# Zokrates/ZoKrates

Measured on NVIDIA H100. Metric: groth16_constraints_per_sec, higher is better.
Workload: dtype u256-montgomery

## Files before the change

zokrates_b200/csrc/ec.cuh:

```cuda
#pragma once
#include "fp2.cuh"

namespace zkb {

template <class F>
struct Affine {
  F x, y;
  ZKB_HD bool is_inf() const { return x.is_zero() && y.is_zero(); }
  ZKB_HD static Affine inf() { return Affine{F::zero(), F::zero()}; }
  ZKB_HD static Affine neg(const Affine& p) { return Affine{p.x, F::neg(p.y)}; }
};

template <class F>
struct XYZZ {
  F x, y, zz, zzz;

  ZKB_HD static XYZZ identity() { return XYZZ{F::zero(), F::zero(), F::zero(), F::zero()}; }
  ZKB_HD bool is_identity() const { return zz.is_zero(); }
  ZKB_HD static XYZZ from_affine(const Affine<F>& p) {
    if (p.is_inf()) return identity();
    return XYZZ{p.x, p.y, F::one(), F::one()};
  }
  ZKB_HD static XYZZ neg(const XYZZ& p) { return XYZZ{p.x, F::neg(p.y), p.zz, p.zzz}; }

  ZKB_HD static XYZZ mdbl(const Affine<F>& p) {
    F U = F::dbl(p.y);
    F V = F::sqr(U);
    F W = F::mul(U, V);
    F S = F::mul(p.x, V);
    F X2 = F::sqr(p.x);
    F M = F::add(F::dbl(X2), X2);
    F X3 = F::sub(F::sqr(M), F::dbl(S));
    F Y3 = F::sub(F::mul(M, F::sub(S, X3)), F::mul(W, p.y));
    return XYZZ{X3, Y3, V, W};
  }

  ZKB_HD static XYZZ dbl(const XYZZ& p) {
    F U = F::dbl(p.y);
    F V = F::sqr(U);
    F W = F::mul(U, V);
    F S = F::mul(p.x, V);
    F X2 = F::sqr(p.x);
    F M = F::add(F::dbl(X2), X2);
    F X3 = F::sub(F::sqr(M), F::dbl(S));
    F Y3 = F::sub(F::mul(M, F::sub(S, X3)), F::mul(W, p.y));
    return XYZZ{X3, Y3, F::mul(V, p.zz), F::mul(W, p.zzz)};
  }

  ZKB_HD static XYZZ madd(const XYZZ& a, const Affine<F>& q) {
    if (q.is_inf()) return a;
    if (a.is_identity()) return XYZZ{q.x, q.y, F::one(), F::one()};
    F U2 = F::mul(q.x, a.zz);
    F S2 = F::mul(q.y, a.zzz);
    F Pd = F::sub(U2, a.x);
    F Rd = F::sub(S2, a.y);
    if (Pd.is_zero()) {
      if (Rd.is_zero()) return mdbl_ni(q);
      return identity();
    }
    F PP = F::sqr(Pd);
    F PPP = F::mul(Pd, PP);
    F Q = F::mul(a.x, PP);
    F X3 = F::sub(F::sub(F::sqr(Rd), PPP), F::dbl(Q));
    F Y3 = F::sub(F::mul(Rd, F::sub(Q, X3)), F::mul(a.y, PPP));
    return XYZZ{X3, Y3, F::mul(a.zz, PP), F::mul(a.zzz, PPP)};
  }

  ZKB_HD static XYZZ add(const XYZZ& a, const XYZZ& b) {
    if (b.is_identity()) return a;
    if (a.is_identity()) return b;
    F U1 = F::mul(a.x, b.zz);
    F U2 = F::mul(b.x, a.zz);
    F S1 = F::mul(a.y, b.zzz);
    F S2 = F::mul(b.y, a.zzz);
    F Pd = F::sub(U2, U1);
    F Rd = F::sub(S2, S1);
    if (Pd.is_zero()) {
      if (Rd.is_zero()) return dbl_ni(a);
      return identity();
    }
    F PP = F::sqr(Pd);
    F PPP = F::mul(Pd, PP);
    F Q = F::mul(U1, PP);
    F X3 = F::sub(F::sub(F::sqr(Rd), PPP), F::dbl(Q));
    F Y3 = F::sub(F::mul(Rd, F::sub(Q, X3)), F::mul(S1, PPP));
    return XYZZ{X3, Y3, F::mul(F::mul(a.zz, b.zz), PP), F::mul(F::mul(a.zzz, b.zzz), PPP)};
  }

  ZKB_NI static XYZZ mdbl_ni(const Affine<F>& p) { return mdbl(p); }
  ZKB_NI static XYZZ dbl_ni(const XYZZ& p) { return dbl(p); }
  ZKB_NI static XYZZ add_ni(const XYZZ& a, const XYZZ& b) { return add(a, b); }
  ZKB_NI static XYZZ madd_ni(const XYZZ& a, const Affine<F>& q) { return madd(a, q); }

  ZKB_NI static Affine<F> to_affine(const XYZZ& p) {
    if (p.is_identity()) return Affine<F>::inf();
    F t = F::inv(F::mul(p.zz, p.zzz));
    F zzi = F::mul(t, p.zzz);
    F zzzi = F::mul(t, p.zz);
    return Affine<F>{F::mul(p.x, zzi), F::mul(p.y, zzzi)};
  }

  ZKB_NI static XYZZ mul_affine(const Affine<F>& base, const uint32_t* k, int nlimbs) {
    XYZZ r = identity();
    for (int i = nlimbs - 1; i >= 0; i--)
      for (int b = 31; b >= 0; b--) {
        r = dbl_ni(r);
        if ((k[i] >> b) & 1) r = madd_ni(r, base);
      }
    return r;
  }
  ZKB_NI static XYZZ mul_xyzz(const XYZZ& base, const uint32_t* k, int nlimbs) {
    XYZZ r = identity();
    for (int i = nlimbs - 1; i >= 0; i--)
      for (int b = 31; b >= 0; b--) {
        r = dbl_ni(r);
        if ((k[i] >> b) & 1) r = add_ni(r, base);
      }
    return r;
  }
};

}
```

zokrates_b200/csrc/fp.cuh:

```cuda
#pragma once
#include "hd.cuh"
#include "field_params.cuh"

namespace zkb {

template <class P>
struct alignas(16) Fp {
  static constexpr int N = P::N;
  typedef P Params;
  uint32_t v[N];

  ZKB_HD static Fp zero() {
    Fp r;
#pragma unroll
    for (int i = 0; i < N; i++) r.v[i] = 0;
    return r;
  }
  ZKB_HD static Fp one() {
    Fp r;
#pragma unroll
    for (int i = 0; i < N; i++) r.v[i] = P::r1(i);
    return r;
  }
  ZKB_HD static Fp r2() {
    Fp r;
#pragma unroll
    for (int i = 0; i < N; i++) r.v[i] = P::r2(i);
    return r;
  }
  ZKB_HD static Fp modulus() {
    Fp r;
#pragma unroll
    for (int i = 0; i < N; i++) r.v[i] = P::mod(i);
    return r;
  }
  ZKB_HD bool is_zero() const {
    uint32_t acc = 0;
#pragma unroll
    for (int i = 0; i < N; i++) acc |= v[i];
    return acc == 0;
  }
  ZKB_HD bool operator==(const Fp& o) const {
    uint32_t acc = 0;
#pragma unroll
    for (int i = 0; i < N; i++) acc |= v[i] ^ o.v[i];
    return acc == 0;
  }
  ZKB_HD bool operator!=(const Fp& o) const { return !(*this == o); }

  ZKB_HD static Fp reduce_once(const Fp& a) {
    Fp t;
    t.v[0] = ptx::sub_cc(a.v[0], P::mod(0));
#pragma unroll
    for (int i = 1; i < N; i++) t.v[i] = ptx::subc_cc(a.v[i], P::mod(i));
    uint32_t borrow = ptx::subc(0, 0);
    Fp r;
#pragma unroll
    for (int i = 0; i < N; i++) r.v[i] = borrow ? a.v[i] : t.v[i];
    return r;
  }

  ZKB_HD static Fp add(const Fp& a, const Fp& b) {
    Fp t;
    t.v[0] = ptx::add_cc(a.v[0], b.v[0]);
#pragma unroll
    for (int i = 1; i < N - 1; i++) t.v[i] = ptx::addc_cc(a.v[i], b.v[i]);
    t.v[N - 1] = ptx::addc(a.v[N - 1], b.v[N - 1]);
    return reduce_once(t);
  }

  ZKB_HD static Fp sub(const Fp& a, const Fp& b) {
    Fp t;
    t.v[0] = ptx::sub_cc(a.v[0], b.v[0]);
#pragma unroll
    for (int i = 1; i < N; i++) t.v[i] = ptx::subc_cc(a.v[i], b.v[i]);
    uint32_t borrow = ptx::subc(0, 0);
    Fp r;
    r.v[0] = ptx::add_cc(t.v[0], P::mod(0) & borrow);
#pragma unroll
    for (int i = 1; i < N - 1; i++) r.v[i] = ptx::addc_cc(t.v[i], P::mod(i) & borrow);
    r.v[N - 1] = ptx::addc(t.v[N - 1], P::mod(N - 1) & borrow);
    return r;
  }

  ZKB_HD static Fp neg(const Fp& a) {
    if (a.is_zero()) return a;
    Fp r;
    r.v[0] = ptx::sub_cc(P::mod(0), a.v[0]);
#pragma unroll
    for (int i = 1; i < N - 1; i++) r.v[i] = ptx::subc_cc(P::mod(i), a.v[i]);
    r.v[N - 1] = ptx::subc(P::mod(N - 1), a.v[N - 1]);
    return r;
  }

  ZKB_HD static Fp dbl(const Fp& a) { return add(a, a); }

  ZKB_HD static Fp mul(const Fp& a, const Fp& b) {
    static_assert(N % 2 == 0, "even limb count");
    uint32_t E[N], O[N];
    {
      const uint32_t y = b.v[0];
#pragma unroll
      for (int j = 0; j < N; j += 2) {
        uint64_t w = (uint64_t)a.v[j] * y;
        E[j] = (uint32_t)w;
        E[j + 1] = (uint32_t)(w >> 32);
        uint64_t u = (uint64_t)a.v[j + 1] * y;
        O[j] = (uint32_t)u;
        O[j + 1] = (uint32_t)(u >> 32);
      }
    }
#pragma unroll
    for (int i = 0; i < N; i++) {
      if (i > 0) {
        const uint32_t y = b.v[i];
        uint32_t nE[N], nO[N];
        nE[0] = ptx::add_cc(O[0], E[1]);
#pragma unroll
        for (int j = 1; j < N - 1; j += 2) ptx::madc_wide_cc(nO[j - 1], nO[j], a.v[j], y, E[j + 1], E[j + 2]);
        ptx::madc_wide(nO[N - 2], nO[N - 1], a.v[N - 1], y, 0, 0);
        ptx::mad_wide_cc(nE[0], nE[1], a.v[0], y, nE[0], O[1]);
#pragma unroll
        for (int j = 2; j < N; j += 2) ptx::madc_wide_cc(nE[j], nE[j + 1], a.v[j], y, O[j], O[j + 1]);
        nO[N - 1] = ptx::addc(nO[N - 1], 0);
#pragma unroll
        for (int j = 0; j < N; j++) {
          E[j] = nE[j];
          O[j] = nO[j];
        }
      }
      const uint32_t m = E[0] * P::INV;
      ptx::mad_wide_cc(O[0], O[1], P::mod(1), m, O[0], O[1]);
#pragma unroll
      for (int j = 3; j < N; j += 2) ptx::madc_wide_cc(O[j - 1], O[j], P::mod(j), m, O[j - 1], O[j]);
      ptx::mad_wide_cc(E[0], E[1], P::mod(0), m, E[0], E[1]);
#pragma unroll
      for (int j = 2; j < N; j += 2) ptx::madc_wide_cc(E[j], E[j + 1], P::mod(j), m, E[j], E[j + 1]);
      O[N - 1] = ptx::addc(O[N - 1], 0);
    }
    Fp t;
    t.v[0] = ptx::add_cc(O[0], E[1]);
#pragma unroll
    for (int k = 1; k < N - 1; k++) t.v[k] = ptx::addc_cc(O[k], E[k + 1]);
    t.v[N - 1] = ptx::addc(O[N - 1], 0);
    return reduce_once(t);
  }

  ZKB_HD static Fp sqr(const Fp& a) { return mul(a, a); }
  ZKB_NI static Fp mul_ni(const Fp& a, const Fp& b) { return mul(a, b); }

  ZKB_HD static Fp to_mont(const Fp& a) { return mul(a, r2()); }
  ZKB_HD static Fp from_mont(const Fp& a) {
    Fp o = zero();
    o.v[0] = 1;
    return mul(a, o);
  }

  ZKB_NI static Fp pow_limbs(const Fp& a, const uint32_t* e, int nlimbs) {
    Fp r = one();
    bool started = false;
    for (int i = nlimbs - 1; i >= 0; i--) {
      for (int b = 31; b >= 0; b--) {
        if (started) r = mul_ni(r, r);
        if ((e[i] >> b) & 1) {
          r = started ? mul_ni(r, a) : a;
          started = true;
        }
      }
    }
    return r;
  }

  ZKB_NI static Fp inv(const Fp& a) {
    uint32_t e[N];
#pragma unroll
    for (int i = 0; i < N; i++) e[i] = P::pm2(i);
    return pow_limbs(a, e, N);
  }

  ZKB_NI static Fp pow_u64(const Fp& a, uint64_t k) {
    uint32_t e[2] = {(uint32_t)k, (uint32_t)(k >> 32)};
    return pow_limbs(a, e, 2);
  }
};

}
```

zokrates_b200/csrc/fp2.cuh:

```cuda
#pragma once
#include "fp.cuh"

namespace zkb {

template <class Bt>
struct Fp2T {
  typedef Bt B;
  typedef Fp2T Fp2;
  B c0, c1;

  ZKB_HD static Fp2 zero() { return Fp2{B::zero(), B::zero()}; }
  ZKB_HD static Fp2 one() { return Fp2{B::one(), B::zero()}; }
  ZKB_HD bool is_zero() const { return c0.is_zero() && c1.is_zero(); }
  ZKB_HD bool operator==(const Fp2& o) const { return c0 == o.c0 && c1 == o.c1; }
  ZKB_HD bool operator!=(const Fp2& o) const { return !(*this == o); }
  ZKB_HD static Fp2 add(const Fp2& a, const Fp2& b) { return Fp2{B::add(a.c0, b.c0), B::add(a.c1, b.c1)}; }
  ZKB_HD static Fp2 sub(const Fp2& a, const Fp2& b) { return Fp2{B::sub(a.c0, b.c0), B::sub(a.c1, b.c1)}; }
  ZKB_HD static Fp2 neg(const Fp2& a) { return Fp2{B::neg(a.c0), B::neg(a.c1)}; }
  ZKB_HD static Fp2 dbl(const Fp2& a) { return Fp2{B::dbl(a.c0), B::dbl(a.c1)}; }
  ZKB_NI static Fp2 mul_v(Fp2 a, Fp2 b) {
    B v0 = B::mul(a.c0, b.c0);
    B v1 = B::mul(a.c1, b.c1);
    B s = B::mul(B::add(a.c0, a.c1), B::add(b.c0, b.c1));
    return Fp2{B::sub(v0, v1), B::sub(B::sub(s, v0), v1)};
  }
  ZKB_NI static Fp2 sqr_v(Fp2 a) {
    B t = B::mul(a.c0, a.c1);
    B r0 = B::mul(B::add(a.c0, a.c1), B::sub(a.c0, a.c1));
    return Fp2{r0, B::dbl(t)};
  }
  ZKB_HD static Fp2 mul(const Fp2& a, const Fp2& b) { return mul_v(a, b); }
  ZKB_HD static Fp2 sqr(const Fp2& a) { return sqr_v(a); }
  ZKB_HD static Fp2 mul_ni(const Fp2& a, const Fp2& b) { return mul_v(a, b); }
  ZKB_NI static Fp2 inv(const Fp2& a) {
    B d = B::inv(B::add(B::sqr(a.c0), B::sqr(a.c1)));
    return Fp2{B::mul(a.c0, d), B::neg(B::mul(a.c1, d))};
  }
  ZKB_HD static Fp2 to_mont(const Fp2& a) { return Fp2{B::to_mont(a.c0), B::to_mont(a.c1)}; }
  ZKB_HD static Fp2 from_mont(const Fp2& a) { return Fp2{B::from_mont(a.c0), B::from_mont(a.c1)}; }
};

template <class P>
using Fp2 = Fp2T<Fp<P>>;

}
```

zokrates_b200/csrc/fp64.cuh:

```cuda
#pragma once
#include "fp.cuh"

namespace zkb {

template <class P>
struct alignas(16) Fp64 {
  static constexpr int N = P::N / 2;
  typedef P Params;
  typedef unsigned __int128 u128;
  uint64_t v[N];

  ZKB_HD static uint64_t modl(int i) { return ((uint64_t)P::mod(2 * i + 1) << 32) | P::mod(2 * i); }
  ZKB_HD static uint64_t inv64() {
    uint64_t p0 = modl(0);
    uint64_t x = (uint64_t)(uint32_t)(0u - P::INV);
    x = x * (2 - p0 * x);
    return (uint64_t)0 - x;
  }
  ZKB_HD static Fp64 zero() { Fp64 r; for (int i = 0; i < N; i++) r.v[i] = 0; return r; }
  ZKB_HD static Fp64 one() { Fp64 r; for (int i = 0; i < N; i++) r.v[i] = ((uint64_t)P::r1(2 * i + 1) << 32) | P::r1(2 * i); return r; }
  ZKB_HD static Fp64 r2() { Fp64 r; for (int i = 0; i < N; i++) r.v[i] = ((uint64_t)P::r2(2 * i + 1) << 32) | P::r2(2 * i); return r; }
  ZKB_HD bool is_zero() const { uint64_t a = 0; for (int i = 0; i < N; i++) a |= v[i]; return a == 0; }
  ZKB_HD bool operator==(const Fp64& o) const { uint64_t a = 0; for (int i = 0; i < N; i++) a |= v[i] ^ o.v[i]; return a == 0; }
  ZKB_HD bool operator!=(const Fp64& o) const { return !(*this == o); }
  ZKB_HD static bool geq_p(const Fp64& a) {
    for (int i = N - 1; i >= 0; i--) { uint64_t m = modl(i); if (a.v[i] > m) return true; if (a.v[i] < m) return false; }
    return true;
  }
  ZKB_HD static Fp64 sub_p(const Fp64& a) {
    Fp64 r; uint64_t borrow = 0;
    for (int i = 0; i < N; i++) { u128 d = (u128)a.v[i] - modl(i) - borrow; r.v[i] = (uint64_t)d; borrow = (uint64_t)(d >> 64) & 1; }
    return r;
  }
  ZKB_HD static Fp64 add(const Fp64& a, const Fp64& b) {
    Fp64 t; uint64_t c = 0;
    for (int i = 0; i < N; i++) { u128 s = (u128)a.v[i] + b.v[i] + c; t.v[i] = (uint64_t)s; c = (uint64_t)(s >> 64); }
    return (c || geq_p(t)) ? sub_p(t) : t;
  }
  ZKB_HD static Fp64 sub(const Fp64& a, const Fp64& b) {
    Fp64 t; uint64_t borrow = 0;
    for (int i = 0; i < N; i++) { u128 d = (u128)a.v[i] - b.v[i] - borrow; t.v[i] = (uint64_t)d; borrow = (uint64_t)(d >> 64) & 1; }
    if (borrow) { uint64_t c = 0; for (int i = 0; i < N; i++) { u128 s = (u128)t.v[i] + modl(i) + c; t.v[i] = (uint64_t)s; c = (uint64_t)(s >> 64); } }
    return t;
  }
  ZKB_HD static Fp64 neg(const Fp64& a) { return a.is_zero() ? a : sub(zero(), a); }
  ZKB_HD static Fp64 dbl(const Fp64& a) { return add(a, a); }
  ZKB_HD static Fp64 mul(const Fp64& a, const Fp64& b) {
    uint64_t t[N + 2];
    for (int i = 0; i < N + 2; i++) t[i] = 0;
    const uint64_t inv = inv64();
    for (int i = 0; i < N; i++) {
      uint64_t c = 0;
      for (int j = 0; j < N; j++) { u128 s = (u128)a.v[j] * b.v[i] + t[j] + c; t[j] = (uint64_t)s; c = (uint64_t)(s >> 64); }
      u128 s2 = (u128)t[N] + c; t[N] = (uint64_t)s2; t[N + 1] = (uint64_t)(s2 >> 64);
      uint64_t m = t[0] * inv;
      u128 s = (u128)m * modl(0) + t[0]; c = (uint64_t)(s >> 64);
      for (int j = 1; j < N; j++) { s = (u128)m * modl(j) + t[j] + c; t[j - 1] = (uint64_t)s; c = (uint64_t)(s >> 64); }
      s2 = (u128)t[N] + c; t[N - 1] = (uint64_t)s2; t[N] = t[N + 1] + (uint64_t)(s2 >> 64);
    }
    Fp64 o; for (int i = 0; i < N; i++) o.v[i] = t[i];
    return (t[N] || geq_p(o)) ? sub_p(o) : o;
  }
  ZKB_HD static Fp64 sqr(const Fp64& a) { return mul(a, a); }
  ZKB_HD static Fp64 mul_ni(const Fp64& a, const Fp64& b) { return mul(a, b); }
  ZKB_HD static Fp64 to_mont(const Fp64& a) { return mul(a, r2()); }
  ZKB_HD static Fp64 from_mont(const Fp64& a) { Fp64 o = zero(); o.v[0] = 1; return mul(a, o); }
  ZKB_HD static Fp64 inv(const Fp64& a) {
    uint64_t e[N];
    for (int i = 0; i < N; i++) e[i] = modl(i);
    uint64_t borrow = 2;
    for (int i = 0; i < N && borrow; i++) { uint64_t o = e[i]; e[i] = o - borrow; borrow = o < borrow ? 1 : 0; }
    Fp64 r = one();
    bool started = false;
    for (int i = N - 1; i >= 0; i--)
      for (int b = 63; b >= 0; b--) {
        if (started) r = mul(r, r);
        if ((e[i] >> b) & 1) { r = started ? mul(r, a) : a; started = true; }
      }
    return r;
  }
};

}
```

Before: 49.40 million.

## Add lazy Montgomery reduction with wide products, dedicated squaring, and fused mul-sub

Splits Montgomery multiplication into a double-width product and a separate REDC, and adds a dedicated squaring that computes the cross terms once and doubles them. EC point addition computes Y3 as a single reduction of a*b - c*d, and Fp2 multiplication (Karatsuba) defers reduction using unreduced sums and a precomputed multiple of p^2. Together these save REDC passes and modular add/sub corrections in the MSM inner loops. This depends on the modulus having two spare top bits (BN254 does), and the new wide code paths add register pressure.

```diff
diff --git a/zokrates_b200/csrc/ec.cuh b/zokrates_b200/csrc/ec.cuh
--- a/zokrates_b200/csrc/ec.cuh
+++ b/zokrates_b200/csrc/ec.cuh
@@ -62,7 +62,7 @@
     F PPP = F::mul(Pd, PP);
     F Q = F::mul(a.x, PP);
     F X3 = F::sub(F::sub(F::sqr(Rd), PPP), F::dbl(Q));
-    F Y3 = F::sub(F::mul(Rd, F::sub(Q, X3)), F::mul(a.y, PPP));
+    F Y3 = F::mul_sub(Rd, F::sub(Q, X3), a.y, PPP);
     return XYZZ{X3, Y3, F::mul(a.zz, PP), F::mul(a.zzz, PPP)};
   }
 
@@ -83,7 +83,7 @@
     F PPP = F::mul(Pd, PP);
     F Q = F::mul(U1, PP);
     F X3 = F::sub(F::sub(F::sqr(Rd), PPP), F::dbl(Q));
-    F Y3 = F::sub(F::mul(Rd, F::sub(Q, X3)), F::mul(S1, PPP));
+    F Y3 = F::mul_sub(Rd, F::sub(Q, X3), S1, PPP);
     return XYZZ{X3, Y3, F::mul(F::mul(a.zz, b.zz), PP), F::mul(F::mul(a.zzz, b.zzz), PPP)};
   }
 
diff --git a/zokrates_b200/csrc/fp.cuh b/zokrates_b200/csrc/fp.cuh
--- a/zokrates_b200/csrc/fp.cuh
+++ b/zokrates_b200/csrc/fp.cuh
@@ -146,7 +146,184 @@
     return reduce_once(t);
   }
 
-  ZKB_HD static Fp sqr(const Fp& a) { return mul(a, a); }
+  static constexpr bool LAZY_HEADROOM = (P::mod(N - 1) >> 30) == 0;
+  struct Wide {
+    uint32_t v[2 * N];
+  };
+
+  template <int M>
+  struct PSq {
+    uint32_t v[2 * N];
+    ZKB_HD constexpr PSq() : v() {
+      for (int i = 0; i < N; i++) {
+        uint64_t c = 0;
+        for (int j = 0; j < N; j++) {
+          uint64_t t = (uint64_t)P::mod(i) * P::mod(j) + v[i + j] + c;
+          v[i + j] = (uint32_t)t;
+          c = t >> 32;
+        }
+        v[i + N] = (uint32_t)c;
+      }
+      uint64_t c = 0;
+      for (int k = 0; k < 2 * N; k++) {
+        uint64_t t = (uint64_t)v[k] * M + c;
+        v[k] = (uint32_t)t;
+        c = t >> 32;
+      }
+    }
+  };
+
+  template <int SIZE>
+  ZKB_HD static void mad_row(uint32_t (&acc)[SIZE], int s, const uint32_t* x, int j0, int cnt, uint32_t y) {
+#pragma unroll
+    for (int t = 0; t < cnt; t++) {
+      const int k = s + 2 * t;
+      if (t == 0)
+        ptx::mad_wide_cc(acc[k], acc[k + 1], x[j0], y, acc[k], acc[k + 1]);
+      else
+        ptx::madc_wide_cc(acc[k], acc[k + 1], x[j0 + 2 * t], y, acc[k], acc[k + 1]);
+    }
+    if (cnt > 0 && s + 2 * cnt < SIZE) acc[s + 2 * cnt] = ptx::addc(acc[s + 2 * cnt], 0);
+  }
+
+  ZKB_HD static Wide merge_eo(const uint32_t (&E)[2 * N], const uint32_t (&O)[2 * N]) {
+    Wide r;
+    r.v[0] = E[0];
+    r.v[1] = ptx::add_cc(E[1], O[0]);
+#pragma unroll
+    for (int k = 2; k < 2 * N - 1; k++) r.v[k] = ptx::addc_cc(E[k], O[k - 1]);
+    r.v[2 * N - 1] = ptx::addc(E[2 * N - 1], O[2 * N - 2]);
+    return r;
+  }
+
+  ZKB_HD static Wide mul_wide(const Fp& a, const Fp& b) {
+    static_assert(N % 2 == 0, "even limb count");
+    uint32_t E[2 * N], O[2 * N];
+#pragma unroll
+    for (int k = 0; k < 2 * N; k++) E[k] = O[k] = 0;
+#pragma unroll
+    for (int i = 0; i < N; i++) {
+      if (i % 2 == 0) {
+        mad_row(E, i, a.v, 0, N / 2, b.v[i]);
+        mad_row(O, i, a.v, 1, N / 2, b.v[i]);
+      } else {
+        mad_row(O, i - 1, a.v, 0, N / 2, b.v[i]);
+        mad_row(E, i + 1, a.v, 1, N / 2, b.v[i]);
+      }
+    }
+    return merge_eo(E, O);
+  }
+
+  ZKB_HD static Wide sqr_wide(const Fp& a) {
+    uint32_t E[2 * N], O[2 * N];
+#pragma unroll
+    for (int k = 0; k < 2 * N; k++) E[k] = O[k] = 0;
+#pragma unroll
+    for (int i = 0; i < N - 1; i++) {
+      mad_row(O, 2 * i, a.v, i + 1, (N - i) / 2, a.v[i]);
+      mad_row(E, 2 * i + 2, a.v, i + 2, (N - 1 - i) / 2, a.v[i]);
+    }
+    Wide t = merge_eo(E, O);
+    Wide r;
+    r.v[0] = 0;
+#pragma unroll
+    for (int k = 2 * N - 1; k >= 1; k--) r.v[k] = (t.v[k] << 1) | (t.v[k - 1] >> 31);
+    ptx::mad_wide_cc(r.v[0], r.v[1], a.v[0], a.v[0], r.v[0], r.v[1]);
+#pragma unroll
+    for (int i = 1; i < N; i++) ptx::madc_wide_cc(r.v[2 * i], r.v[2 * i + 1], a.v[i], a.v[i], r.v[2 * i], r.v[2 * i + 1]);
+    return r;
+  }
+
+  ZKB_HD static Fp redc(const Wide& T) {
+    uint32_t E[N], O[N];
+#pragma unroll
+    for (int j = 0; j < N; j++) {
+      E[j] = T.v[j];
+      O[j] = 0;
+    }
+    {
+      const uint32_t m = E[0] * P::INV;
+      ptx::mad_wide_cc(O[0], O[1], P::mod(1), m, O[0], O[1]);
+#pragma unroll
+      for (int j = 3; j < N; j += 2) ptx::madc_wide_cc(O[j - 1], O[j], P::mod(j), m, O[j - 1], O[j]);
+      ptx::mad_wide_cc(E[0], E[1], P::mod(0), m, E[0], E[1]);
+#pragma unroll
+      for (int j = 2; j < N; j += 2) ptx::madc_wide_cc(E[j], E[j + 1], P::mod(j), m, E[j], E[j + 1]);
+      O[N - 1] = ptx::addc(O[N - 1], 0);
+    }
+#pragma unroll
+    for (int i = 1; i < N; i++) {
+      uint32_t nE[N], nO[N];
+      nE[0] = ptx::add_cc(O[0], E[1]);
+      const uint32_t m = nE[0] * P::INV;
+#pragma unroll
+      for (int j = 1; j < N - 1; j += 2) ptx::madc_wide_cc(nO[j - 1], nO[j], P::mod(j), m, E[j + 1], E[j + 2]);
+      ptx::madc_wide(nO[N - 2], nO[N - 1], P::mod(N - 1), m, 0, 0);
+      ptx::mad_wide_cc(nE[0], nE[1], P::mod(0), m, nE[0], O[1]);
+#pragma unroll
+      for (int j = 2; j < N; j += 2) ptx::madc_wide_cc(nE[j], nE[j + 1], P::mod(j), m, O[j], O[j + 1]);
+      nO[N - 1] = ptx::addc(nO[N - 1], 0);
+#pragma unroll
+      for (int j = 0; j < N; j++) {
+        E[j] = nE[j];
+        O[j] = nO[j];
+      }
+    }
+    Fp t;
+    t.v[0] = ptx::add_cc(O[0], E[1]);
+#pragma unroll
+    for (int k = 1; k < N - 1; k++) t.v[k] = ptx::addc_cc(O[k], E[k + 1]);
+    t.v[N - 1] = ptx::addc(O[N - 1], 0);
+    t.v[0] = ptx::add_cc(t.v[0], T.v[N]);
+#pragma unroll
+    for (int k = 1; k < N - 1; k++) t.v[k] = ptx::addc_cc(t.v[k], T.v[N + k]);
+    t.v[N - 1] = ptx::addc(t.v[N - 1], T.v[2 * N - 1]);
+    return reduce_once(t);
+  }
+
+  ZKB_HD static Wide add_wide(const Wide& a, const Wide& b) {
+    Wide r;
+    r.v[0] = ptx::add_cc(a.v[0], b.v[0]);
+#pragma unroll
+    for (int k = 1; k < 2 * N - 1; k++) r.v[k] = ptx::addc_cc(a.v[k], b.v[k]);
+    r.v[2 * N - 1] = ptx::addc(a.v[2 * N - 1], b.v[2 * N - 1]);
+    return r;
+  }
+  ZKB_HD static Wide sub_wide(const Wide& a, const Wide& b) {
+    Wide r;
+    r.v[0] = ptx::sub_cc(a.v[0], b.v[0]);
+#pragma unroll
+    for (int k = 1; k < 2 * N - 1; k++) r.v[k] = ptx::subc_cc(a.v[k], b.v[k]);
+    r.v[2 * N - 1] = ptx::subc(a.v[2 * N - 1], b.v[2 * N - 1]);
+    return r;
+  }
+  template <int M>
+  ZKB_HD static Wide add_psq(const Wide& a) {
+    static_assert(LAZY_HEADROOM && M <= 2, "M p^2 plus the operand must stay < p*R");
+    constexpr PSq<M> K{};
+    Wide r;
+    r.v[0] = ptx::add_cc(a.v[0], K.v[0]);
+#pragma unroll
+    for (int i = 1; i < 2 * N - 1; i++) r.v[i] = ptx::addc_cc(a.v[i], K.v[i]);
+    r.v[2 * N - 1] = ptx::addc(a.v[2 * N - 1], K.v[2 * N - 1]);
+    return r;
+  }
+  ZKB_HD static Fp add_nr(const Fp& a, const Fp& b) {
+    static_assert(LAZY_HEADROOM, "a product of two unreduced sums (< 4p^2) must stay < p*R");
+    Fp t;
+    t.v[0] = ptx::add_cc(a.v[0], b.v[0]);
+#pragma unroll
+    for (int i = 1; i < N - 1; i++) t.v[i] = ptx::addc_cc(a.v[i], b.v[i]);
+    t.v[N - 1] = ptx::addc(a.v[N - 1], b.v[N - 1]);
+    return t;
+  }
+
+  ZKB_HD static Fp mul_sub(const Fp& a, const Fp& b, const Fp& c, const Fp& d) {
+    static_assert(LAZY_HEADROOM, "a sum of two products (< 2p^2) must stay < p*R");
+    return redc(add_wide(mul_wide(a, b), mul_wide(c, neg(d))));
+  }
+
+  ZKB_HD static Fp sqr(const Fp& a) { return redc(sqr_wide(a)); }
   ZKB_NI static Fp mul_ni(const Fp& a, const Fp& b) { return mul(a, b); }
 
   ZKB_HD static Fp to_mont(const Fp& a) { return mul(a, r2()); }
diff --git a/zokrates_b200/csrc/fp2.cuh b/zokrates_b200/csrc/fp2.cuh
--- a/zokrates_b200/csrc/fp2.cuh
+++ b/zokrates_b200/csrc/fp2.cuh
@@ -19,16 +19,42 @@
   ZKB_HD static Fp2 neg(const Fp2& a) { return Fp2{B::neg(a.c0), B::neg(a.c1)}; }
   ZKB_HD static Fp2 dbl(const Fp2& a) { return Fp2{B::dbl(a.c0), B::dbl(a.c1)}; }
   ZKB_NI static Fp2 mul_v(Fp2 a, Fp2 b) {
-    B v0 = B::mul(a.c0, b.c0);
-    B v1 = B::mul(a.c1, b.c1);
-    B s = B::mul(B::add(a.c0, a.c1), B::add(b.c0, b.c1));
-    return Fp2{B::sub(v0, v1), B::sub(B::sub(s, v0), v1)};
+    if constexpr (!B::LAZY_HEADROOM) {
+      B v0 = B::mul(a.c0, b.c0), v1 = B::mul(a.c1, b.c1);
+      B s = B::mul(B::add(a.c0, a.c1), B::add(b.c0, b.c1));
+      return Fp2{B::sub(v0, v1), B::sub(B::sub(s, v0), v1)};
+    } else {
+      typedef typename B::Wide Wd;
+      Wd v0 = B::mul_wide(a.c0, b.c0);
+      Wd v1 = B::mul_wide(a.c1, b.c1);
+      Wd s = B::mul_wide(B::add_nr(a.c0, a.c1), B::add_nr(b.c0, b.c1));
+      B c1 = B::redc(B::sub_wide(B::sub_wide(s, v0), v1));
+      B c0 = B::redc(B::sub_wide(B::template add_psq<1>(v0), v1));
+      return Fp2{c0, c1};
+    }
   }
   ZKB_NI static Fp2 sqr_v(Fp2 a) {
-    B t = B::mul(a.c0, a.c1);
-    B r0 = B::mul(B::add(a.c0, a.c1), B::sub(a.c0, a.c1));
-    return Fp2{r0, B::dbl(t)};
+    B r0 = B::mul(B::add_nr(a.c0, a.c1), B::sub(a.c0, a.c1));
+    B r1 = B::mul(B::add_nr(a.c0, a.c0), a.c1);
+    return Fp2{r0, r1};
   }
+  ZKB_NI static Fp2 mul_sub_v(Fp2 a, Fp2 b, Fp2 c, Fp2 d) {
+    if constexpr (!B::LAZY_HEADROOM) {
+      return sub(mul_v(a, b), mul_v(c, d));
+    } else {
+      typedef typename B::Wide Wd;
+      Fp2 e = neg(d);
+      Wd v0 = B::mul_wide(a.c0, b.c0);
+      Wd w0 = B::mul_wide(c.c0, e.c0);
+      Wd v1 = B::add_wide(B::mul_wide(a.c1, b.c1), B::mul_wide(c.c1, e.c1));
+      Wd s = B::add_wide(B::mul_wide(B::add_nr(a.c0, a.c1), B::add_nr(b.c0, b.c1)),
+                         B::mul_wide(B::add_nr(c.c0, c.c1), B::add_nr(e.c0, e.c1)));
+      B c1 = B::redc(B::sub_wide(B::sub_wide(B::sub_wide(s, v0), w0), v1));
+      B c0 = B::redc(B::sub_wide(B::template add_psq<2>(B::add_wide(v0, w0)), v1));
+      return Fp2{c0, c1};
+    }
+  }
+  ZKB_HD static Fp2 mul_sub(const Fp2& a, const Fp2& b, const Fp2& c, const Fp2& d) { return mul_sub_v(a, b, c, d); }
   ZKB_HD static Fp2 mul(const Fp2& a, const Fp2& b) { return mul_v(a, b); }
   ZKB_HD static Fp2 sqr(const Fp2& a) { return sqr_v(a); }
   ZKB_HD static Fp2 mul_ni(const Fp2& a, const Fp2& b) { return mul_v(a, b); }
diff --git a/zokrates_b200/csrc/fp64.cuh b/zokrates_b200/csrc/fp64.cuh
--- a/zokrates_b200/csrc/fp64.cuh
+++ b/zokrates_b200/csrc/fp64.cuh
@@ -62,6 +62,9 @@
     return (t[N] || geq_p(o)) ? sub_p(o) : o;
   }
   ZKB_HD static Fp64 sqr(const Fp64& a) { return mul(a, a); }
+  static constexpr bool LAZY_HEADROOM = false;
+  ZKB_HD static Fp64 add_nr(const Fp64& a, const Fp64& b) { return add(a, b); }
+  ZKB_HD static Fp64 mul_sub(const Fp64& a, const Fp64& b, const Fp64& c, const Fp64& d) { return sub(mul(a, b), mul(c, d)); }
   ZKB_HD static Fp64 mul_ni(const Fp64& a, const Fp64& b) { return mul(a, b); }
   ZKB_HD static Fp64 to_mont(const Fp64& a) { return mul(a, r2()); }
   ZKB_HD static Fp64 from_mont(const Fp64& a) { Fp64 o = zero(); o.v[0] = 1; return mul(a, o); }
```

Result: faster. 52.04 million (median of 6 runs) (+5.3%).
